# google-deepmind/open_spiel

Hardware: NVIDIA H100
Metric: connect_four ApplyAction env steps/sec (batched) (higher is better)
Workload: dtype u64

## Files before the change

### open_spiel_b200/csrc/api.cu

```cuda
#include <ctype.h>
#include <math.h>
#include <sched.h>
#include <stdlib.h>
#include <stdio.h>
#include <string.h>

#include <memory>
#include <mutex>
#include <string>
#include <vector>

#include "batch_kernels.cuh"
#include "errors.h"

namespace b2s {

long long g_launches = 0;
static thread_local std::string g_err;

int fail(const std::string& m) { g_err = m; return 1; }
int cuda_fail(cudaError_t e, const char* what) {
  g_err = std::string(what) + ": " + cudaGetErrorString(e);
  return 2;
}
#define CU(x) do { cudaError_t _e = (x); if (_e != cudaSuccess) return cuda_fail(_e, #x); } while (0)

constexpr int kMaxDevices = 64;
struct HostPipe {
  std::mutex mu;
  cudaStream_t hs = nullptr, hs2 = nullptr;
  cudaEvent_t ev[8] = {};
};
// ... 134 lines not shown
  if (count == 0) return fail("bind: no CPUs listed in " + path);
  if (sched_setaffinity(0, sizeof set, &set) != 0) return fail("bind: sched_setaffinity failed");
  if (n_cpus) *n_cpus = count;
  return 0;
}

int b2s_device_count(void) {
  int n = 0;
  if (cudaGetDeviceCount(&n) != cudaSuccess) { cudaGetLastError(); return 0; }
  return n;
}

int b2s_batch_create(int game_id, const b2s_params* params, int64_t capacity, int device, void** out_batch) {
  if (!out_batch) return fail("null out_batch");
  *out_batch = nullptr;
  if (capacity <= 0) return fail("capacity must be positive");
  if (b2s_device_count() <= 0) return fail("no CUDA device: the b2s device path has no CPU fallback");
  GameOps* ops = make_ops(game_id, params);
  if (!ops) return fail("unsupported game id");
  b2s_params p;
  if (params) p = *params; else b2s_params_default(&p);
  Batch* B = new Batch;
  B->ops = ops;
  memset(&B->info, 0, sizeof B->info);
  const char* e = ops->configure(p, B->info);
  if (e) { delete B; return fail(e); }
  B->cap = capacity;
  B->device = device;
  cudaError_t ce = cudaSetDevice(device);
  if (ce != cudaSuccess) { delete B; return cuda_fail(ce, "cudaSetDevice"); }
  ops->device_init();
  ce = cudaGetLastError();
  if (ce != cudaSuccess) { delete B; return cuda_fail(ce, "per-game device tables"); }
  size_t bytes = ops->chunk_bytes() * (size_t)ops->chunks() * (size_t)capacity;
  ce = cudaMalloc(&B->planes, bytes);
  if (ce != cudaSuccess) { delete B; return cuda_fail(ce, "cudaMalloc(state planes)"); }
  if (B->info.history_bytes > 0) {
    ce = cudaMalloc((void**)&B->hist, (size_t)B->info.history_bytes * (size_t)capacity);
    if (ce != cudaSuccess) { delete B; return cuda_fail(ce, "cudaMalloc(history)"); }
  }
  ce = cudaMalloc((void**)&B->err, sizeof(ErrBuf));
  if (ce != cudaSuccess) { delete B; return cuda_fail(ce, "cudaMalloc(err)"); }
  ops->reset(B->ctx(), capacity, 0);
  ce = cudaDeviceSynchronize();
  if (ce != cudaSuccess) { delete B; return cuda_fail(ce, "initial reset"); }
  *out_batch = B;
  return 0;
}

void b2s_batch_destroy(void* batch) {
  if (!batch) return;
  Batch* B = (Batch*)batch;
  cudaSetDevice(B->device);
  delete B;
}

int b2s_batch_info(void* batch, b2s_game_info* out) {
  if (!batch || !out) return fail("null argument");
  *out = ((Batch*)batch)->info;
  return 0;
}
int64_t b2s_batch_capacity(void* batch) { return batch ? ((Batch*)batch)->cap : 0; }

int b2s_reset(void* batch, int64_t n, void* stream) {
  if (int r = check(batch, n)) return r;
  Batch* B = (Batch*)batch;
  B->ops->reset(B->ctx(), n, (cudaStream_t)stream);
// ... 36 lines not shown
  Batch* B = (Batch*)batch;
  if (!obs_d) return fail("null obs");
  if ((uintptr_t)obs_d & 3u) return fail("observation: output pointer must be 4-byte aligned");
  if (player >= B->info.num_players) return fail("player out of range");
  const char* e = B->ops->obs(B->ctx(), player, 0, 0, obs_d, n, (cudaStream_t)stream);
  if (e) return fail(e);
  return post();
}

int b2s_information_state(void* batch, int player, float* out_d, int64_t n, void* stream) {
  if (int r = check(batch, n)) return r;
  Batch* B = (Batch*)batch;
  if (!out_d) return fail("null out");
  if ((uintptr_t)out_d & 3u) return fail("information_state: output pointer must be 4-byte aligned");
  if (player >= B->info.num_players) return fail("player out of range");
  const char* e = B->ops->obs(B->ctx(), player, 1, 0, out_d, n, (cudaStream_t)stream);
  if (e) return fail(e);
  return post();
}

int b2s_step_fused(void* batch, const int32_t* actions_d, uint32_t* mask_d, uint8_t* term_d, float* rets_d, int64_t n, void* stream) {
  if (int r = check(batch, n)) return r;
  if (!actions_d) return fail("null actions");
  Batch* B = (Batch*)batch;
  B->ops->step_fused(B->ctx(), actions_d, mask_d, term_d, rets_d, n, (cudaStream_t)stream);
  return post();
}

constexpr size_t kHostGraphsPerBatch = 4;

static int enqueue_host_step(Batch* B, HostPipe& pipe, const void* actions_h, int action_bytes, uint32_t* mask_h, uint8_t* term_or_status_h,
                             float* rets_h, int64_t n, int compact, int n_chunks, bool join) {
  cudaStream_t st = pipe.hs, st2 = pipe.hs2;
  const size_t W = (size_t)B->info.mask_words, P = (size_t)B->info.num_players, cb = B->ops->chunk_bytes();
  const size_t ab = (size_t)action_bytes;
  const int64_t chunk = n_chunks > 1 ? ((n + n_chunks - 1) / n_chunks + 1023) / 1024 * 1024 : n;
  int c = 0, rc = 0;
  cudaError_t e = cudaSuccess;
  for (int64_t lo = 0; lo < n && !rc; lo += chunk, ++c) {
    const int64_t len = n - lo < chunk ? n - lo : chunk;
    Ctx v = B->ctx();
    v.planes = (char*)v.planes + (size_t)lo * cb;
    if (v.hist) v.hist += lo;
    v.lane0 = lo;
    char* act_d = (char*)B->act_d + (size_t)lo * ab;
    e = cudaMemcpyAsync(act_d, (const char*)actions_h + (size_t)lo * ab, ab * len, cudaMemcpyHostToDevice, st);
    if (e != cudaSuccess) { rc = cuda_fail(e, "step_host: upload"); break; }
    if (compact)
      B->ops->step_compact(v, act_d, action_bytes, B->term_d + lo, mask_h ? B->mask_d + lo * W : nullptr, len, st);
    else
      B->ops->step_fused(v, (const int*)act_d, mask_h ? B->mask_d + lo * W : nullptr, term_or_status_h ? B->term_d + lo : nullptr,
                         rets_h ? B->rets_d + lo * P : nullptr, len, st);
    if ((rc = post())) break;
    cudaEvent_t ev = pipe.ev[c % kHostChunks];
    if ((e = cudaEventRecord(ev, st)) != cudaSuccess || (e = cudaStreamWaitEvent(st2, ev, 0)) != cudaSuccess) { rc = cuda_fail(e, "step_host: event"); break; }
    if (mask_h && (e = cudaMemcpyAsync(mask_h + lo * W, B->mask_d + lo * W, sizeof(u32) * W * len, cudaMemcpyDeviceToHost, st2)) != cudaSuccess) { rc = cuda_fail(e, "step_host: download"); break; }
    if (term_or_status_h && (e = cudaMemcpyAsync(term_or_status_h + lo, B->term_d + lo, len, cudaMemcpyDeviceToHost, st2)) != cudaSuccess) { rc = cuda_fail(e, "step_host: download"); break; }
    if (rets_h && (e = cudaMemcpyAsync(rets_h + lo * P, B->rets_d + lo * P, sizeof(float) * P * len, cudaMemcpyDeviceToHost, st2)) != cudaSuccess) { rc = cuda_fail(e, "step_host: download"); break; }
  }
  if (join && c > 0) {
    cudaEvent_t ev = pipe.ev[c % kHostChunks];
    if ((e = cudaEventRecord(ev, st2)) != cudaSuccess || (e = cudaStreamWaitEvent(st, ev, 0)) != cudaSuccess) { if (!rc) rc = cuda_fail(e, "step_host: join"); }
  }
  return rc;
}

static int step_host_impl(Batch* B, const void* actions_h, int action_bytes, uint32_t* mask_h, uint8_t* term_or_status_h,
                          float* rets_h, int64_t n, int compact) {
  if (B->device < 0 || B->device >= kMaxDevices) return fail("device index out of range");
  HostPipe& pipe = g_host_pipe[B->device];
  std::lock_guard<std::mutex> lock(pipe.mu);
  if (!pipe.hs) {
    CU(cudaStreamCreateWithFlags(&pipe.hs, cudaStreamDefault));
    CU(cudaStreamCreateWithFlags(&pipe.hs2, cudaStreamDefault));
    for (int i = 0; i < kHostChunks; ++i) CU(cudaEventCreateWithFlags(&pipe.ev[i], cudaEventDisableTiming));
// ... 105 lines not shown
}

int b2s_step_fused_host_compact(void* batch, const void* actions_h, int action_bytes, uint8_t* status_h, uint32_t* mask_h, int64_t n) {
  if (int r = check(batch, n)) return r;
  if (!actions_h || !status_h) return fail("null actions / status");
  Batch* B = (Batch*)batch;
  if (action_bytes != 1 && action_bytes != 4) return fail("step_compact: action_bytes must be 1 (uint8, 0xFF = skip) or 4 (int32, -1 = skip)");
  if (action_bytes == 1 && B->info.num_distinct_actions > 255) return fail("step_compact: uint8 actions need num_distinct_actions <= 255");
  if (B->info.min_utility != -1.0 || B->info.max_utility != 1.0 || B->info.max_chance_outcomes > 0)
    return fail("step_compact: the 2-bit outcome code needs a win / loss / draw game (use b2s_step_fused_host)");
  return step_host_impl(B, actions_h, action_bytes, mask_h, status_h, nullptr, n, 1);
}

int b2s_error_count(void* batch, int64_t* count, int64_t* first_bad_lane, void* stream) {
  if (int r = check(batch, 0)) return r;
  Batch* B = (Batch*)batch;
  ErrBuf e;
  CU(cudaMemcpyAsync(&e, B->err, sizeof e, cudaMemcpyDeviceToHost, (cudaStream_t)stream));
  CU(cudaStreamSynchronize((cudaStream_t)stream));
  if (count) *count = (int64_t)e.count;
  if (first_bad_lane) *first_bad_lane = e.count ? e.first : -1;
  return 0;
}

int b2s_state_get(void* batch, int64_t idx, void* host_blob, size_t cap) {
  if (int r = check(batch, 0)) return r;
  Batch* B = (Batch*)batch;
  if (idx < 0 || idx >= B->cap) return fail("lane out of range");
  size_t cb = B->ops->chunk_bytes(), sb = (size_t)B->info.state_bytes;
  size_t need = sb + B->info.history_bytes;
  if (cap < need) return fail("blob too small");
  CU(cudaDeviceSynchronize());
  std::vector<uint4> stored((cb * B->ops->chunks() + 15) / 16), blob((sb + 15) / 16);
  for (int k = 0; k < B->ops->chunks(); ++k)
    CU(cudaMemcpy((char*)stored.data() + k * cb, (char*)B->planes + ((size_t)k * B->cap + idx) * cb, cb, cudaMemcpyDeviceToHost));
  B->ops->stored_to_blob(stored.data(), blob.data());
  char* out = (char*)host_blob;
  memcpy(out, blob.data(), sb);
  if (B->info.history_bytes)
    CU(cudaMemcpy2D(out + sb, sizeof(u64), B->hist + idx, sizeof(u64) * B->cap, sizeof(u64),
                    B->info.history_bytes / sizeof(u64), cudaMemcpyDeviceToHost));
  return 0;
}
int b2s_state_set(void* batch, int64_t idx, const void* host_blob, size_t len) {
  if (int r = check(batch, 0)) return r;
  Batch* B = (Batch*)batch;
  if (idx < 0 || idx >= B->cap) return fail("lane out of range");
  size_t cb = B->ops->chunk_bytes(), sb = (size_t)B->info.state_bytes;
  size_t need = sb + B->info.history_bytes;
  if (len != need) return fail("blob size mismatch");
  CU(cudaDeviceSynchronize());
  const char* in = (const char*)host_blob;
  std::vector<uint4> stored((cb * B->ops->chunks() + 15) / 16), blob((sb + 15) / 16);
  memcpy(blob.data(), in, sb);
  B->ops->blob_to_stored(blob.data(), stored.data());
  for (int k = 0; k < B->ops->chunks(); ++k)
    CU(cudaMemcpy((char*)B->planes + ((size_t)k * B->cap + idx) * cb, (const char*)stored.data() + k * cb, cb, cudaMemcpyHostToDevice));
  if (B->info.history_bytes)
    CU(cudaMemcpy2D(B->hist + idx, sizeof(u64) * B->cap, in + sb, sizeof(u64), sizeof(u64),
                    B->info.history_bytes / sizeof(u64), cudaMemcpyHostToDevice));
  return 0;
}

int b2s_broadcast_state(void* dst_batch, int64_t dst_begin, int64_t count, void* src_batch, int64_t src, void* stream) {
  if (int r = check(dst_batch, 0)) return r;
  if (!src_batch) return fail("null src batch");
  Batch* D = (Batch*)dst_batch;
  Batch* S = (Batch*)src_batch;
  if (D->info.game_id != S->info.game_id || D->device != S->device ||
      memcmp(&D->info, &S->info, sizeof(b2s_game_info)) != 0)
    return fail("broadcast: batches differ in game/params/device");
  if (dst_begin < 0 || count < 0 || dst_begin + count > D->cap || src < 0 || src >= S->cap) return fail("broadcast: range");
  D->ops->broadcast(D->ctx(), dst_begin, count, S->ctx(), src, (cudaStream_t)stream);
  return post();
}

int b2s_copy_states(void* dst_batch, int64_t dst_begin, void* src_batch, int64_t src_begin, int64_t count, void* stream) {
  if (int r = check(dst_batch, 0)) return r;
  if (!src_batch) return fail("null src batch");
  Batch* D = (Batch*)dst_batch;
  Batch* S = (Batch*)src_batch;
  if (D->device != S->device || memcmp(&D->info, &S->info, sizeof(b2s_game_info)) != 0)
    return fail("copy: batches differ in game/params/device");
  if (dst_begin < 0 || src_begin < 0 || count < 0 || dst_begin + count > D->cap || src_begin + count > S->cap)
    return fail("copy: range");
  D->ops->copy(D->ctx(), dst_begin, S->ctx(), src_begin, count, (cudaStream_t)stream);
  return post();
}

int b2s_rollout(void* batch, uint64_t seed, int64_t lane_offset, int64_t n, float* rets_d, int32_t* plies_d, void* stream) {
// ... 315 lines not shown
```

### open_spiel_b200/csrc/batch_kernels.cuh

```cuda
#pragma once
#include <new>
#include <string.h>

#include "common.cuh"

namespace b2s {

constexpr int kBlock = 256;

extern long long g_launches;

__device__ __forceinline__ void pdl_wait() { asm volatile("griddepcontrol.wait;" ::: "memory"); }
__device__ __forceinline__ void pdl_launch_dependents() { asm volatile("griddepcontrol.launch_dependents;" ::: "memory"); }

template <typename... KArgs, typename... Args>
inline void launch_pdl(void (*kernel)(KArgs...), unsigned grid, cudaStream_t st, Args... args) {
  cudaLaunchConfig_t cfg = {};
  cfg.gridDim = dim3(grid);
  cfg.blockDim = dim3(kBlock);
  cfg.stream = st;
  cudaLaunchAttribute at[1];
  at[0].id = cudaLaunchAttributeProgrammaticStreamSerialization;
  at[0].val.programmaticStreamSerializationAllowed = 1;
  cfg.attrs = at;
  cfg.numAttrs = 1;
  cudaLaunchKernelEx(&cfg, kernel, static_cast<KArgs>(args)...);
}


template <class R>
__global__ void __launch_bounds__(kBlock) k_reset(Ctx ctx, typename R::Cfg cfg, long long n) {
  long long i = (long long)blockIdx.x * kBlock + threadIdx.x;
  if (i == 0) { ctx.err->count = 0; ctx.err->first = 0x7fffffffffffffffLL; }
  if (i >= n) return;
  typename R::S s;
  R::init(s, cfg, ctx, i);
  store_state<R>(s, cfg, ctx, i);
}

template <class R, int ILP>
__global__ void __launch_bounds__(kBlock, R::kMinBlocks) k_apply(Ctx ctx, typename R::Cfg cfg, const int* __restrict__ actions, long long n) {
  pdl_wait();
  long long base = (long long)blockIdx.x * (kBlock * ILP) + threadIdx.x;
  int a[ILP];
  Fetched<R> pk[ILP];
#pragma unroll
  for (int j = 0; j < ILP; ++j) {
    long long i = base + (long long)j * kBlock;
    a[j] = -1;
    if (i < n) { a[j] = __ldg(actions + i); fetch_state<R>(pk[j], ctx, i); }
  }
  pdl_launch_dependents();
#pragma unroll
  for (int j = 0; j < ILP; ++j) {
    long long i = base + (long long)j * kBlock;
    if (a[j] == -1) continue;
    typename R::S s;
    unpack_state<R>(s, pk[j], cfg);
    if (R::terminal(s, cfg) || !R::apply(s, a[j], cfg, ctx, i)) { flag_error(ctx.err, ctx.lane0 + i); continue; }
    store_state<R>(s, cfg, ctx, i);
  }
}

template <int MAXW>
struct MaskStage {
  static constexpr int kRow = MAXW | 1;
  u32 w[kBlock / 32][32 * kRow];
};
template <int MAXW>
__device__ __forceinline__ void store_masks_coalesced(u32* __restrict__ mask, long long first, long long n, bool active, int W,
                                                      const u32* m, MaskStage<MAXW>& stage) {
  const int lane = threadIdx.x & 31;
  u32* st = stage.w[threadIdx.x >> 5];
  if (active) {
#pragma unroll
    for (int k = 0; k < MAXW; ++k) if (k < W) st[lane * MaskStage<MAXW>::kRow + k] = m[k];
  }
  __syncwarp();
  const long long left = n - first;
  const int total = (int)(left < 32 ? left : 32) * W;
  int q = lane / W, r = lane - q * W;
  const int dq = 32 / W, dr = 32 - dq * W;
  u32* out = mask + first * W;
  for (int f = lane; f < total; f += 32) {
    out[f] = st[q * MaskStage<MAXW>::kRow + r];
    q += dq; r += dr;
    if (r >= W) { r -= W; ++q; }
  }
  __syncwarp();
}

template <class R, int ILP>
__global__ void __launch_bounds__(kBlock) k_legal_mask(Ctx ctx, typename R::Cfg cfg, u32* __restrict__ mask, int mask_words, long long n) {
  long long base = (long long)blockIdx.x * (kBlock * ILP) + threadIdx.x;
  Fetched<R> pk[ILP];
#pragma unroll
  for (int j = 0; j < ILP; ++j) {
    long long i = base + (long long)j * kBlock;
    if (i < n) fetch_state<R>(pk[j], ctx, i);
  }
  __shared__ MaskStage<R::kMaskWords == 1 ? 0 : R::kMaskWords> stage;
#pragma unroll
  for (int j = 0; j < ILP; ++j) {
    long long i = base + (long long)j * kBlock;
    u32 m[R::kMaskWords];
    if (i < n) {
      typename R::S s;
      unpack_state<R>(s, pk[j], cfg);
      R::legal(s, cfg, m);
    }
    if (R::kMaskWords == 1) {
      if (i < n) mask[i] = m[0];
    } else {
      store_masks_coalesced(mask, i - (threadIdx.x & 31), n, i < n, mask_words, m, stage);
    }
  }
}

template <class R>
__global__ void __launch_bounds__(kBlock) k_legal_list(Ctx ctx, typename R::Cfg cfg, short* __restrict__ out, int* __restrict__ counts, int stride, int mask_words, long long n) {
  long long i = (long long)blockIdx.x * kBlock + threadIdx.x;
  if (i >= n) return;
  typename R::S s;
  load_state<R>(s, cfg, ctx, i);
  u32 m[R::kMaskWords];
  R::legal(s, cfg, m);
  int k = 0;
  for (int w = 0; w < mask_words; ++w) {
    u32 bits = m[w];
    while (bits) {
      int b = __ffs(bits) - 1;
      bits &= bits - 1;
      if (k < stride) out[i * stride + k] = (short)(w * 32 + b);
      ++k;
    }
  }
  counts[i] = k;
}

template <class R, int ILP>
__global__ void __launch_bounds__(kBlock) k_status(Ctx ctx, typename R::Cfg cfg, signed char* __restrict__ cur, unsigned char* __restrict__ term, float* __restrict__ rets, long long n) {
  long long base = (long long)blockIdx.x * (kBlock * ILP) + threadIdx.x;
  Fetched<R> pk[ILP];
#pragma unroll
  for (int j = 0; j < ILP; ++j) {
    long long i = base + (long long)j * kBlock;
    if (i < n) fetch_state<R>(pk[j], ctx, i);
  }
#pragma unroll
  for (int j = 0; j < ILP; ++j) {
    long long i = base + (long long)j * kBlock;
    if (i >= n) continue;
    typename R::S s;
    unpack_state<R>(s, pk[j], cfg);
    int cp = R::cur_player(s, cfg);
    if (cur) cur[i] = (signed char)cp;
    if (term) term[i] = cp == kTerminalPlayerId ? 1 : 0;
    if (rets) {
      float r[R::kPlayers];
      R::returns(s, cfg, r);
      if (R::kPlayers == 2) reinterpret_cast<float2*>(rets)[i] = make_float2(r[0], r[1]);
      else { const int np = rule_num_players<R>(cfg); for (int p = 0; p < np; ++p) rets[i * np + p] = r[p]; }
    }
  }
}

template <class R, int ILP>
__global__ void __launch_bounds__(kBlock) k_step_fused(Ctx ctx, typename R::Cfg cfg, const int* __restrict__ actions, u32* __restrict__ mask, int mask_words, unsigned char* __restrict__ term, float* __restrict__ rets, long long n) {
  pdl_wait();
  long long base = (long long)blockIdx.x * (kBlock * ILP) + threadIdx.x;
  int a[ILP];
  Fetched<R> pk[ILP];
#pragma unroll
  for (int j = 0; j < ILP; ++j) {
    long long i = base + (long long)j * kBlock;
    a[j] = -1;
    if (i < n) { a[j] = __ldg(actions + i); fetch_state<R>(pk[j], ctx, i); }
  }
  pdl_launch_dependents();
  __shared__ MaskStage<R::kMaskWords == 1 ? 0 : R::kMaskWords> stage;
#pragma unroll
  for (int j = 0; j < ILP; ++j) {
    long long i = base + (long long)j * kBlock;
    const bool live = i < n;
    u32 m[R::kMaskWords];
    if (live) {
      typename R::S s;
      unpack_state<R>(s, pk[j], cfg);
      if (a[j] != -1) {
        if (R::terminal(s, cfg) || !R::apply(s, a[j], cfg, ctx, i)) flag_error(ctx.err, ctx.lane0 + i);
        else store_state<R>(s, cfg, ctx, i);
      }
      bool t = R::terminal(s, cfg);
      if (term) term[i] = t ? 1 : 0;
      if (rets) {
        float r[R::kPlayers];
        R::returns(s, cfg, r);
        if (R::kPlayers == 2) reinterpret_cast<float2*>(rets)[i] = make_float2(r[0], r[1]);
        else { const int np = rule_num_players<R>(cfg); for (int p = 0; p < np; ++p) rets[i * np + p] = r[p]; }
      }
      if (mask) {
        if (t) { for (int w = 0; w < R::kMaskWords; ++w) m[w] = 0; }
        else R::legal_nonterminal(s, cfg, m);
      }
    }
    if (mask) {
      if (R::kMaskWords == 1) { if (live) mask[i] = m[0]; }
      else store_masks_coalesced(mask, i - (threadIdx.x & 31), n, live, mask_words, m, stage);
    }
  }
}

template <class R, int ILP, class AT>
__global__ void __launch_bounds__(kBlock) k_step_compact(Ctx ctx, typename R::Cfg cfg, const AT* __restrict__ actions, unsigned char* __restrict__ status,
                                                         u32* __restrict__ mask, int mask_words, int small_mask, long long n) {
  pdl_wait();
  long long base = (long long)blockIdx.x * (kBlock * ILP) + threadIdx.x;
  int a[ILP];
  Fetched<R> pk[ILP];
#pragma unroll
  for (int j = 0; j < ILP; ++j) {
    long long i = base + (long long)j * kBlock;
    a[j] = -1;
    if (i < n) {
      AT raw = __ldg(actions + i);
      a[j] = (sizeof(AT) == 1 && (unsigned char)raw == 0xFFu) ? -1 : (int)raw;
      fetch_state<R>(pk[j], ctx, i);
    }
  }
  pdl_launch_dependents();
  __shared__ MaskStage<R::kMaskWords == 1 ? 0 : R::kMaskWords> stage;
#pragma unroll
  for (int j = 0; j < ILP; ++j) {
    long long i = base + (long long)j * kBlock;
    const bool live = i < n;
    u32 m[R::kMaskWords];
    if (live) {
      typename R::S s;
      unpack_state<R>(s, pk[j], cfg);
      if (a[j] != -1) {
        if (R::terminal(s, cfg) || !R::apply(s, a[j], cfg, ctx, i)) flag_error(ctx.err, ctx.lane0 + i);
        else store_state<R>(s, cfg, ctx, i);
// ... 269 lines not shown
__global__ void __launch_bounds__(kBlock) k_copy_to_blob(Ctx dst, Ctx srcctx, long long count, typename R::Cfg cfg) {
  long long i = (long long)blockIdx.x * kBlock + threadIdx.x;
  if (i >= count) return;
  typename R::S s;
  load_state<R>(s, cfg, srcctx, i);
  R::store(s, dst, i);
  R::copy_history(dst, i, srcctx, i, s, cfg);
}

template <class R>
__global__ void __launch_bounds__(kBlock) k_gather(Ctx dst, Ctx srcctx, const long long* __restrict__ src_lanes, long long count, typename R::Cfg cfg) {
  long long i = (long long)blockIdx.x * kBlock + threadIdx.x;
  if (i >= count) return;
  long long sl = src_lanes[i];
  if (sl < 0 || sl >= srcctx.cap) { flag_error(dst.err, i); return; }
  typename R::S s;
  load_state<R>(s, cfg, srcctx, sl);
  store_state<R>(s, cfg, dst, i);
  R::copy_history(dst, i, srcctx, sl, s, cfg);
}


struct Batch;

template <class R> auto call_device_init(int) -> decltype(R::device_init(), void()) { R::device_init(); }
template <class R> void call_device_init(long) {}

struct GameOps {
  virtual ~GameOps() {}
  virtual void device_init() = 0;
  virtual const char* configure(const b2s_params& p, b2s_game_info& gi) = 0;
  virtual size_t chunk_bytes() const = 0;
  virtual int chunks() const = 0;
  virtual void stored_to_blob(const void* stored, void* blob) const = 0;
  virtual void blob_to_stored(const void* blob, void* stored) const = 0;
  virtual void reset(const Ctx&, long long n, cudaStream_t) = 0;
  virtual void apply(const Ctx&, const int* a, long long n, cudaStream_t) = 0;
  virtual void legal_mask(const Ctx&, u32* m, long long n, cudaStream_t) = 0;
  virtual void legal_list(const Ctx&, short* out, int* counts, int stride, long long n, cudaStream_t) = 0;
  virtual void status(const Ctx&, signed char* cur, unsigned char* term, float* rets, long long n, cudaStream_t) = 0;
  virtual const char* obs(const Ctx&, int player, int which, int zero_terminal, float* out, long long n, cudaStream_t) = 0;
  virtual void step_fused(const Ctx&, const int* a, u32* m, unsigned char* term, float* rets, long long n, cudaStream_t) = 0;
  virtual void step_compact(const Ctx&, const void* a, int action_bytes, unsigned char* status, u32* m, long long n, cudaStream_t) = 0;
  virtual void step_compact_zero_copy(const Ctx&, const unsigned char* a_host, unsigned char* status_host, long long n, cudaStream_t) = 0;
  virtual void rollout(const Ctx&, u64 seed, long long lane_offset, float* rets, int* plies, long long n, cudaStream_t) = 0;
  virtual void broadcast(const Ctx& dst, long long dst0, long long count, const Ctx& src, long long srclane, cudaStream_t) = 0;
  virtual void copy(const Ctx& dst, long long dst0, const Ctx& src, long long src0, long long count, cudaStream_t) = 0;
  virtual void copy_to_blob(const Ctx& dst, const Ctx& src, long long count, cudaStream_t) = 0;
  virtual void gather(const Ctx& dst, const Ctx& src, const long long* src_lanes, long long count, cudaStream_t) = 0;
  virtual void traj_begin(const Ctx&, u64 seed, long long lane_offset, int* lengths, long long n, cudaStream_t) = 0;
  virtual void traj_step(const Ctx&, u64 seed, long long lane_offset, int t, const TrajStepOut& o, long long n, cudaStream_t) = 0;
  virtual void traj_finish(const Ctx&, float* rewards, long long n, cudaStream_t) = 0;
  virtual const char* mcts(const Ctx& roots, const Ctx& work, long long n, const struct MctsArgs& args, cudaStream_t) = 0;
  virtual const char* mcts_eval_limits(int* max_legal, int* max_path) const = 0;
  virtual void mcts_eval_step(const Ctx& roots, const Ctx& leaves, long long n, const struct MctsEvalArgs& args, cudaStream_t) = 0;
  virtual void mcts_eval_report(long long n, const struct MctsEvalArgs& args, cudaStream_t) = 0;
  b2s_game_info info;
};

template <class R, class Q = typename R::Packed>
void stored_to_blob_impl(const typename R::Cfg& c, const void* stored, void* blob, int) {
  typename R::S s;
  R::unpack(s, *static_cast<const Q*>(stored), c);
  Ctx b = {};
  b.planes = blob; b.cap = 1;
  R::store(s, b, 0);
// ... 11 lines not shown
template <class R>
void blob_to_stored_impl(const typename R::Cfg&, const void* blob, void* stored, long) { memcpy(stored, blob, sizeof(typename R::Chunk) * R::kChunks); }

inline unsigned grid_for(long long n, int ilp = 1) { return (unsigned)((n + (long long)kBlock * ilp - 1) / ((long long)kBlock * ilp)); }

inline bool make_magic(int d, int limit, u32* out) {
  u64 M = ((1ull << 32) + d - 1) / d;
  if (M >> 32) { if (d == 1) { *out = 0; return false; } }
  for (int e = 0; e < limit; ++e)
    if ((int)(((u64)e * M) >> 32) != e / d) return false;
  *out = (u32)M;
  return true;
}

template <class R>
struct GameOpsT : GameOps {
  typename R::Cfg cfg;
  const char* configure(const b2s_params& p, b2s_game_info& gi) override {
    const char* e = R::make_cfg(p, cfg, gi);
    if (e) return e;
    int width = gi.num_distinct_actions > gi.max_chance_outcomes ? gi.num_distinct_actions : gi.max_chance_outcomes;
    gi.mask_words = (width + 31) / 32;
    if (gi.mask_words > R::kMaskWords) return "action space too large for the device path";
    gi.state_bytes = (int)(sizeof(typename R::Chunk) * R::kChunks);
    gi.game_id = R::kGameId;
    info = gi;
    return nullptr;
  }
  void device_init() override { call_device_init<R>(0); }
  size_t chunk_bytes() const override { return sizeof(StoredChunk<R>); }
  void stored_to_blob(const void* stored, void* blob) const override { stored_to_blob_impl<R>(cfg, stored, blob, 0); }
  void blob_to_stored(const void* blob, void* stored) const override { blob_to_stored_impl<R>(cfg, blob, stored, 0); }
  int chunks() const override { return R::kChunks; }
  void reset(const Ctx& c, long long n, cudaStream_t st) override {
    long long m = n > 0 ? n : 1;
    k_reset<R><<<grid_for(m), kBlock, 0, st>>>(c, cfg, n); ++g_launches;
  }
  void apply(const Ctx& c, const int* a, long long n, cudaStream_t st) override {
    if (n <= 0) return;
    launch_pdl(k_apply<R, R::kIlp>, grid_for(n, R::kIlp), st, c, cfg, a, n); ++g_launches;
  }
  void legal_mask(const Ctx& c, u32* m, long long n, cudaStream_t st) override {
    if (n <= 0) return;
    k_legal_mask<R, R::kIlp><<<grid_for(n, R::kIlp), kBlock, 0, st>>>(c, cfg, m, info.mask_words, n); ++g_launches;
  }
  void legal_list(const Ctx& c, short* out, int* counts, int stride, long long n, cudaStream_t st) override {
    if (n <= 0) return;
    k_legal_list<R><<<grid_for(n), kBlock, 0, st>>>(c, cfg, out, counts, stride, info.mask_words, n); ++g_launches;
  }
  void status(const Ctx& c, signed char* cur, unsigned char* term, float* rets, long long n, cudaStream_t st) override {
    if (n <= 0) return;
    k_status<R, R::kIlp><<<grid_for(n, R::kIlp), kBlock, 0, st>>>(c, cfg, cur, term, rets, n); ++g_launches;
  }
  const char* obs(const Ctx& c, int player, int which, int zero_terminal, float* out, long long n, cudaStream_t st) override {
    int size = which == 0 ? info.observation_tensor_size : info.information_state_tensor_size;
    if (size <= 0) return "game provides no such tensor";
    if (which == 1 && !R::kHasInfoState) return "game provides no information state tensor";
    if (n <= 0) return nullptr;
    u32 magic;
    if (!make_magic(size, 32 * size, &magic)) return "internal: no division magic";
    k_obs<R><<<grid_for(n), kBlock, 0, st>>>(c, cfg, player, which, zero_terminal, out, size, magic, n); ++g_launches;
    return nullptr;
  }
  void step_fused(const Ctx& c, const int* a, u32* m, unsigned char* term, float* rets, long long n, cudaStream_t st) override {
    if (n <= 0) return;
    launch_pdl(k_step_fused<R, R::kIlp>, grid_for(n, R::kIlp), st, c, cfg, a, m, info.mask_words, term, rets, n); ++g_launches;
// ... 126 lines not shown
```

### open_spiel_b200/csrc/common.cuh

```cuda
#pragma once
#include <cuda_runtime.h>
#include <stdint.h>

#include "../../include/b2s.h"

namespace b2s {

typedef unsigned long long u64;
typedef unsigned int u32;

constexpr int kChancePlayerId = -1;
constexpr int kTerminalPlayerId = -4;

struct ErrBuf {
  u64 count;
  long long first;
};

__device__ __forceinline__ void flag_error(ErrBuf* e, long long lane) {
  atomicAdd(&e->count, 1ull);
  atomicMin(&e->first, lane);
}

struct Ctx {
// ... 36 lines not shown
      if ((u32)m >= n || (u32)m >= (u32)(0u - n) % n) return (u32)(m >> 32);
    }
  }
}

__device__ __forceinline__ int nth_set_bit(const u32* words, int nwords, int k) {
  for (int w = 0; w < nwords; ++w) {
    int c = __popc(words[w]);
    if (k < c) return w * 32 + (int)__fns(words[w], 0, k + 1);
    k -= c;
  }
  return -1;
}

template <class R, class S, class Cfg>
__device__ __forceinline__ auto apply_known_legal_impl(S& s, int a, const Cfg& c, const Ctx& ctx, long long lane, int)
    -> decltype(R::apply_legal(s, a, c, ctx, lane)) { return R::apply_legal(s, a, c, ctx, lane); }
template <class R, class S, class Cfg>
__device__ __forceinline__ bool apply_known_legal_impl(S& s, int a, const Cfg& c, const Ctx& ctx, long long lane, long) {
  return R::apply(s, a, c, ctx, lane);
}
template <class R, class S, class Cfg>
__device__ __forceinline__ bool apply_known_legal(S& s, int a, const Cfg& c, const Ctx& ctx, long long lane) {
  return apply_known_legal_impl<R>(s, a, c, ctx, lane, 0);
}

template <class R, class Cfg>
__device__ __forceinline__ auto rule_num_players_impl(const Cfg& c, int) -> decltype(R::num_players(c)) { return R::num_players(c); }
template <class R, class Cfg>
__device__ __forceinline__ int rule_num_players_impl(const Cfg&, long) { return R::kPlayers; }
template <class R, class Cfg>
__device__ __forceinline__ int rule_num_players(const Cfg& c) { return rule_num_players_impl<R>(c, 0); }

template <class R> auto fetched_of(int) -> typename R::Packed;
template <class R> auto fetched_of(long) -> typename R::S;
template <class R> using Fetched = decltype(fetched_of<R>(0));
template <class R> auto stored_of(int) -> typename R::Packed;
template <class R> auto stored_of(long) -> typename R::Chunk;
template <class R> using StoredChunk = decltype(stored_of<R>(0));
template <class R, class P, class Q = typename R::Packed>
__device__ __forceinline__ void fetch_state_impl(P& p, const Ctx& ctx, long long i, int) { p = reinterpret_cast<const Q*>(ctx.planes)[i]; }
template <class R, class P>
__device__ __forceinline__ void fetch_state_impl(P& p, const Ctx& ctx, long long i, long) { R::load(p, ctx, i); }
template <class R, class P>
__device__ __forceinline__ void fetch_state(P& p, const Ctx& ctx, long long i) { fetch_state_impl<R>(p, ctx, i, 0); }
template <class R, class S, class P, class Cfg, class Q = typename R::Packed>
__device__ __forceinline__ void unpack_state_impl(S& s, const P& p, const Cfg& c, int) { R::unpack(s, p, c); }
template <class R, class S, class P, class Cfg>
__device__ __forceinline__ void unpack_state_impl(S& s, const P& p, const Cfg&, long) { s = p; }
template <class R, class S, class P, class Cfg>
__device__ __forceinline__ void unpack_state(S& s, const P& p, const Cfg& c) { unpack_state_impl<R>(s, p, c, 0); }
template <class R, class S, class Cfg, class Q = typename R::Packed>
__device__ __forceinline__ void load_state_impl(S& s, const Cfg& c, const Ctx& ctx, long long i, int) {
  R::unpack(s, reinterpret_cast<const Q*>(ctx.planes)[i], c);
}
template <class R, class S, class Cfg>
__device__ __forceinline__ void load_state_impl(S& s, const Cfg&, const Ctx& ctx, long long i, long) { R::load(s, ctx, i); }
template <class R, class S, class Cfg>
__device__ __forceinline__ void load_state(S& s, const Cfg& c, const Ctx& ctx, long long i) { load_state_impl<R>(s, c, ctx, i, 0); }
template <class R, class S, class Cfg, class Q = typename R::Packed>
__device__ __forceinline__ void store_state_impl(const S& s, const Cfg& c, const Ctx& ctx, long long i, int) {
  reinterpret_cast<Q*>(ctx.planes)[i] = R::pack(s, c);
}
template <class R, class S, class Cfg>
__device__ __forceinline__ void store_state_impl(const S& s, const Cfg&, const Ctx& ctx, long long i, long) { R::store(s, ctx, i); }
template <class R, class S, class Cfg>
__device__ __forceinline__ void store_state(const S& s, const Cfg& c, const Ctx& ctx, long long i) { store_state_impl<R>(s, c, ctx, i, 0); }

template <class R, class S, class Cfg, class Draw>
__device__ __forceinline__ auto playout_step_impl(S& s, const Cfg& c, const Ctx& ctx, long long lane, int ,
                                                  Draw& draw, u32 ply, int) -> decltype(R::num_candidates(s, c)) {
  int n = R::num_candidates(s, c);
  for (u32 retry = 0;; ++retry) {
    int a = R::candidate(s, c, (int)draw(ply + 4096u * retry, (u32)n));
    if (R::play_candidate(s, a, c, ctx, lane)) return a;
  }
}
template <class R, class S, class Cfg, class Draw>
__device__ __forceinline__ int playout_step_impl(S& s, const Cfg& c, const Ctx& ctx, long long lane, int mask_words,
                                                 Draw& draw, u32 ply, long) {
  u32 m[R::kMaskWords];
  R::legal_nonterminal(s, c, m);
  int cnt = 0;
  for (int w = 0; w < mask_words; ++w) cnt += __popc(m[w]);
  int a = nth_set_bit(m, mask_words, (int)draw(ply, (u32)cnt));
  apply_known_legal<R>(s, a, c, ctx, lane);
  return a;
}
template <class R, class S, class Cfg, class Draw>
__device__ __forceinline__ int playout_step(S& s, const Cfg& c, const Ctx& ctx, long long lane, int mask_words, Draw& draw, u32 ply) {
  return playout_step_impl<R>(s, c, ctx, lane, mask_words, draw, ply, 0);
}

struct B128 {
  u64 lo, hi;
// ... 134 lines not shown
```

### open_spiel_b200/csrc/rules_connect_four.cuh

```cuda
#pragma once
#include "common.cuh"

namespace b2s {

template <bool kStd>
struct ConnectFourCore {
  static constexpr int kGameId = B2S_CONNECT_FOUR;
  typedef uint4 Chunk;
  typedef u64 Packed;
  static constexpr int kChunks = 1;
  static constexpr int kMaskWords = 1;
  static constexpr int kObsWords = 3;
  static constexpr int kPlayers = 2;
  static constexpr int kMaxPath = 72;
  static constexpr int kMaxLegal = 32;
  static constexpr int kFilterWords = 0;
  static constexpr int kIlp = 4;
  static constexpr int kMinBlocks = 6;
  static constexpr bool kHasInfoState = false;
  static constexpr int kStdRows = 6, kStdCols = 7, kStdK = 4;

  struct Cfg {
    int rows, cols, k, ego;
    int h1;
    int meta;
    int gather;
    u32 gmul_lo, gmul_hi;
    int gsh_lo, gsh_hi, cols_lo;
    int rgather;
    u32 rmul_lo, rmul_hi;
    int rsh_lo, rsh_hi, rcols_lo, rfirst_hi;
    u64 top;
    u64 board;
    u64 bottom;
    u64 fill[6];
  };
  struct S { u64 x, o; };
  __host__ __device__ static __forceinline__ int ROWS(const Cfg& c) { return kStd ? kStdRows : c.rows; }
  __host__ __device__ static __forceinline__ int COLS(const Cfg& c) { return kStd ? kStdCols : c.cols; }
  __host__ __device__ static __forceinline__ int H1(const Cfg& c) { return kStd ? kStdRows + 1 : c.h1; }
  __host__ __device__ static __forceinline__ int K(const Cfg& c) { return kStd ? kStdK : c.k; }
  __host__ __device__ static __forceinline__ bool META(const Cfg& c) { return kStd ? true : c.meta != 0; }

  static __host__ const char* make_cfg(const b2s_params& p, Cfg& c, b2s_game_info& gi) {
    c.rows = p.rows >= 0 ? p.rows : 6;
    c.cols = p.columns >= 0 ? p.columns : 7;
    c.k = p.x_in_row >= 0 ? p.x_in_row : 4;
    c.ego = p.egocentric_obs_tensor > 0 ? 1 : 0;
    if (c.rows < 1 || c.cols < 1 || c.k < 1) return "connect_four: rows, columns, x_in_row must be positive";
    if ((c.rows + 1) * c.cols > 64 || c.cols > 32)
      return "connect_four: (rows+1)*columns must fit 64 bits for the device path";
    if (kStd && (c.rows != kStdRows || c.cols != kStdCols || c.k != kStdK)) return "connect_four: not the default board";
// ... 234 lines not shown
```

Before: 139.4 billion.

## Store standard connect-four state in 7-byte lane tiles with quad-lane vector access

Standard connect-four states are stored in a tiled layout of 128 lanes per 896 bytes (4-byte low word, 2-byte and 1-byte high planes) instead of 8 bytes per lane. Each thread now owns four consecutive lanes and reads or writes them with vectorized loads and stores for actions, state, masks, terminal flags and returns. The aim is to cut memory traffic in this bandwidth-bound step kernel. In exchange it adds byte-permute pack and unpack work, special handling at the batch tail, and tiled host-side lane read/write paths.

```diff
diff --git a/open_spiel_b200/csrc/api.cu b/open_spiel_b200/csrc/api.cu
--- a/open_spiel_b200/csrc/api.cu
+++ b/open_spiel_b200/csrc/api.cu
@@ -1,3 +1,4 @@
+#include <cassert>
 #include <ctype.h>
 #include <math.h>
 #include <sched.h>
@@ -198,7 +199,7 @@
   ops->device_init();
   ce = cudaGetLastError();
   if (ce != cudaSuccess) { delete B; return cuda_fail(ce, "per-game device tables"); }
-  size_t bytes = ops->chunk_bytes() * (size_t)ops->chunks() * (size_t)capacity;
+  size_t bytes = ops->planes_bytes(capacity);
   ce = cudaMalloc(&B->planes, bytes);
   if (ce != cudaSuccess) { delete B; return cuda_fail(ce, "cudaMalloc(state planes)"); }
   if (B->info.history_bytes > 0) {
@@ -301,7 +302,7 @@
 static int enqueue_host_step(Batch* B, HostPipe& pipe, const void* actions_h, int action_bytes, uint32_t* mask_h, uint8_t* term_or_status_h,
                              float* rets_h, int64_t n, int compact, int n_chunks, bool join) {
   cudaStream_t st = pipe.hs, st2 = pipe.hs2;
-  const size_t W = (size_t)B->info.mask_words, P = (size_t)B->info.num_players, cb = B->ops->chunk_bytes();
+  const size_t W = (size_t)B->info.mask_words, P = (size_t)B->info.num_players;
   const size_t ab = (size_t)action_bytes;
   const int64_t chunk = n_chunks > 1 ? ((n + n_chunks - 1) / n_chunks + 1023) / 1024 * 1024 : n;
   int c = 0, rc = 0;
@@ -309,7 +310,8 @@
   for (int64_t lo = 0; lo < n && !rc; lo += chunk, ++c) {
     const int64_t len = n - lo < chunk ? n - lo : chunk;
     Ctx v = B->ctx();
-    v.planes = (char*)v.planes + (size_t)lo * cb;
+    assert(lo % 1024 == 0);
+    v.planes = (char*)v.planes + B->ops->lane_offset(lo);
     if (v.hist) v.hist += lo;
     v.lane0 = lo;
     char* act_d = (char*)B->act_d + (size_t)lo * ab;
@@ -481,8 +483,7 @@
   if (cap < need) return fail("blob too small");
   CU(cudaDeviceSynchronize());
   std::vector<uint4> stored((cb * B->ops->chunks() + 15) / 16), blob((sb + 15) / 16);
-  for (int k = 0; k < B->ops->chunks(); ++k)
-    CU(cudaMemcpy((char*)stored.data() + k * cb, (char*)B->planes + ((size_t)k * B->cap + idx) * cb, cb, cudaMemcpyDeviceToHost));
+  CU(B->ops->read_lane(B->planes, B->cap, idx, stored.data()));
   B->ops->stored_to_blob(stored.data(), blob.data());
   char* out = (char*)host_blob;
   memcpy(out, blob.data(), sb);
@@ -503,8 +504,7 @@
   std::vector<uint4> stored((cb * B->ops->chunks() + 15) / 16), blob((sb + 15) / 16);
   memcpy(blob.data(), in, sb);
   B->ops->blob_to_stored(blob.data(), stored.data());
-  for (int k = 0; k < B->ops->chunks(); ++k)
-    CU(cudaMemcpy((char*)B->planes + ((size_t)k * B->cap + idx) * cb, (const char*)stored.data() + k * cb, cb, cudaMemcpyHostToDevice));
+  CU(B->ops->write_lane(B->planes, B->cap, idx, stored.data()));
   if (B->info.history_bytes)
     CU(cudaMemcpy2D(B->hist + idx, sizeof(u64) * B->cap, in + sb, sizeof(u64), sizeof(u64),
                     B->info.history_bytes / sizeof(u64), cudaMemcpyHostToDevice));
diff --git a/open_spiel_b200/csrc/batch_kernels.cuh b/open_spiel_b200/csrc/batch_kernels.cuh
--- a/open_spiel_b200/csrc/batch_kernels.cuh
+++ b/open_spiel_b200/csrc/batch_kernels.cuh
@@ -28,6 +28,44 @@
 }
 
 
+template <class AT>
+__device__ __forceinline__ int action_of(AT raw) { return (sizeof(AT) == 1 && (unsigned char)raw == 0xFFu) ? -1 : (int)raw; }
+template <class AT>
+__device__ __forceinline__ void actions4(int a[4], const AT* __restrict__ act, long long i0, long long n) {
+  if (i0 + 4 <= n && ((unsigned long long)(act + i0) & (4 * sizeof(AT) - 1)) == 0) {
+    if constexpr (sizeof(AT) == 4) {
+      const int4 v = __ldg(reinterpret_cast<const int4*>(act + i0));
+      a[0] = v.x; a[1] = v.y; a[2] = v.z; a[3] = v.w;
+    } else {
+      const uchar4 v = __ldg(reinterpret_cast<const uchar4*>(act + i0));
+      a[0] = action_of(v.x); a[1] = action_of(v.y); a[2] = action_of(v.z); a[3] = action_of(v.w);
+    }
+  } else {
+#pragma unroll
+    for (int j = 0; j < 4; ++j) a[j] = i0 + j < n ? action_of(__ldg(act + i0 + j)) : -1;
+  }
+}
+__device__ __forceinline__ void out4(u32* __restrict__ p, long long i0, long long n, const u32 v[4]) {
+  if (i0 + 4 <= n && ((unsigned long long)(p + i0) & 15) == 0) *reinterpret_cast<uint4*>(p + i0) = make_uint4(v[0], v[1], v[2], v[3]);
+  else for (int j = 0; j < 4; ++j) if (i0 + j < n) p[i0 + j] = v[j];
+}
+__device__ __forceinline__ void out4(unsigned char* __restrict__ p, long long i0, long long n, const u32 v[4]) {
+  if (i0 + 4 <= n && ((unsigned long long)(p + i0) & 3) == 0) *reinterpret_cast<u32*>(p + i0) = v[0] | v[1] << 8 | v[2] << 16 | v[3] << 24;
+  else for (int j = 0; j < 4; ++j) if (i0 + j < n) p[i0 + j] = (unsigned char)v[j];
+}
+__device__ __forceinline__ void out4(float2* __restrict__ p, long long i0, long long n, const float2 v[4]) {
+  if (i0 + 4 <= n && ((unsigned long long)(p + i0) & 15) == 0) {
+    reinterpret_cast<float4*>(p + i0)[0] = make_float4(v[0].x, v[0].y, v[1].x, v[1].y);
+    reinterpret_cast<float4*>(p + i0)[1] = make_float4(v[2].x, v[2].y, v[3].x, v[3].y);
+  } else for (int j = 0; j < 4; ++j) if (i0 + j < n) p[i0 + j] = v[j];
+}
+template <class R, int ILP>
+__device__ __forceinline__ long long stream_base() {
+  if constexpr (lane_tiled<R>()) return 4 * ((long long)blockIdx.x * kBlock + threadIdx.x);
+  else return (long long)blockIdx.x * (kBlock * ILP) + threadIdx.x;
+}
+template <class R> constexpr long long stream_stride() { return lane_tiled<R>() ? 1 : kBlock; }
+
 template <class R>
 __global__ void __launch_bounds__(kBlock) k_reset(Ctx ctx, typename R::Cfg cfg, long long n) {
   long long i = (long long)blockIdx.x * kBlock + threadIdx.x;
@@ -40,26 +78,37 @@
 
 template <class R, int ILP>
 __global__ void __launch_bounds__(kBlock, R::kMinBlocks) k_apply(Ctx ctx, typename R::Cfg cfg, const int* __restrict__ actions, long long n) {
+  constexpr bool Q = lane_tiled<R>();
+  static_assert(!Q || ILP == 4, "a thread owns one quad of tiled lanes");
   pdl_wait();
-  long long base = (long long)blockIdx.x * (kBlock * ILP) + threadIdx.x;
+  const long long base = stream_base<R, ILP>();
+  constexpr long long kStride = stream_stride<R>();
   int a[ILP];
   Fetched<R> pk[ILP];
+  if constexpr (Q) {
+    actions4(a, actions, base, n);
+    lanes4_fetch(pk, ctx, base, n);
+  } else {
+#pragma unroll
+    for (int j = 0; j < ILP; ++j) {
+      long long i = base + (long long)j * kStride;
+      a[j] = -1;
+      if (i < n) { a[j] = __ldg(actions + i); fetch_state<R>(pk[j], ctx, i); }
+    }
+  }
+  pdl_launch_dependents();
+  unsigned moved = 0;
 #pragma unroll
   for (int j = 0; j < ILP; ++j) {
-    long long i = base + (long long)j * kBlock;
-    a[j] = -1;
-    if (i < n) { a[j] = __ldg(actions + i); fetch_state<R>(pk[j], ctx, i); }
-  }
-  pdl_launch_dependents();
-#pragma unroll
-  for (int j = 0; j < ILP; ++j) {
-    long long i = base + (long long)j * kBlock;
+    long long i = base + (long long)j * kStride;
     if (a[j] == -1) continue;
     typename R::S s;
     unpack_state<R>(s, pk[j], cfg);
     if (R::terminal(s, cfg) || !R::apply(s, a[j], cfg, ctx, i)) { flag_error(ctx.err, ctx.lane0 + i); continue; }
-    store_state<R>(s, cfg, ctx, i);
-  }
+    if constexpr (Q) { pk[j] = R::pack(s, cfg); moved |= 1u << j; }
+    else store_state<R>(s, cfg, ctx, i);
+  }
+  if constexpr (Q) lanes4_store(pk, moved, ctx, base, n);
 }
 
 template <int MAXW>
@@ -92,29 +141,38 @@
 
 template <class R, int ILP>
 __global__ void __launch_bounds__(kBlock) k_legal_mask(Ctx ctx, typename R::Cfg cfg, u32* __restrict__ mask, int mask_words, long long n) {
-  long long base = (long long)blockIdx.x * (kBlock * ILP) + threadIdx.x;
+  constexpr bool Q = lane_tiled<R>();
+  static_assert(!Q || (ILP == 4 && R::kMaskWords == 1), "a thread owns one quad of tiled lanes");
+  const long long base = stream_base<R, ILP>();
+  constexpr long long kStride = stream_stride<R>();
   Fetched<R> pk[ILP];
+  if constexpr (Q) lanes4_fetch(pk, ctx, base, n);
+  else {
+#pragma unroll
+    for (int j = 0; j < ILP; ++j) {
+      long long i = base + (long long)j * kStride;
+      if (i < n) fetch_state<R>(pk[j], ctx, i);
+    }
+  }
+  __shared__ MaskStage<R::kMaskWords == 1 ? 0 : R::kMaskWords> stage;
+  u32 m4[4];
 #pragma unroll
   for (int j = 0; j < ILP; ++j) {
-    long long i = base + (long long)j * kBlock;
-    if (i < n) fetch_state<R>(pk[j], ctx, i);
-  }
-  __shared__ MaskStage<R::kMaskWords == 1 ? 0 : R::kMaskWords> stage;
-#pragma unroll
-  for (int j = 0; j < ILP; ++j) {
-    long long i = base + (long long)j * kBlock;
+    long long i = base + (long long)j * kStride;
     u32 m[R::kMaskWords];
     if (i < n) {
       typename R::S s;
       unpack_state<R>(s, pk[j], cfg);
       R::legal(s, cfg, m);
     }
-    if (R::kMaskWords == 1) {
+    if constexpr (Q) m4[j] = m[0];
+    else if (R::kMaskWords == 1) {
       if (i < n) mask[i] = m[0];
     } else {
       store_masks_coalesced(mask, i - (threadIdx.x & 31), n, i < n, mask_words, m, stage);
     }
   }
+  if constexpr (Q) out4(mask, base, n, m4);
 }
 
 template <class R>
@@ -140,20 +198,34 @@
 
 template <class R, int ILP>
 __global__ void __launch_bounds__(kBlock) k_status(Ctx ctx, typename R::Cfg cfg, signed char* __restrict__ cur, unsigned char* __restrict__ term, float* __restrict__ rets, long long n) {
-  long long base = (long long)blockIdx.x * (kBlock * ILP) + threadIdx.x;
+  constexpr bool Q = lane_tiled<R>();
+  static_assert(!Q || (ILP == 4 && R::kPlayers == 2), "a thread owns one quad of tiled lanes");
+  const long long base = stream_base<R, ILP>();
+  constexpr long long kStride = stream_stride<R>();
   Fetched<R> pk[ILP];
+  if constexpr (Q) lanes4_fetch(pk, ctx, base, n);
+  else {
+#pragma unroll
+    for (int j = 0; j < ILP; ++j) {
+      long long i = base + (long long)j * kStride;
+      if (i < n) fetch_state<R>(pk[j], ctx, i);
+    }
+  }
+  u32 cp4[4] = {0, 0, 0, 0}, t4[4] = {0, 0, 0, 0};
+  float2 r4[4] = {};
 #pragma unroll
   for (int j = 0; j < ILP; ++j) {
-    long long i = base + (long long)j * kBlock;
-    if (i < n) fetch_state<R>(pk[j], ctx, i);
-  }
-#pragma unroll
-  for (int j = 0; j < ILP; ++j) {
-    long long i = base + (long long)j * kBlock;
+    long long i = base + (long long)j * kStride;
     if (i >= n) continue;
     typename R::S s;
     unpack_state<R>(s, pk[j], cfg);
     int cp = R::cur_player(s, cfg);
+    if constexpr (Q) {
+      cp4[j] = (unsigned char)(signed char)cp; t4[j] = cp == kTerminalPlayerId ? 1 : 0;
+      float r[R::kPlayers];
+      if (rets) { R::returns(s, cfg, r); r4[j] = make_float2(r[0], r[1]); }
+      continue;
+    }
     if (cur) cur[i] = (signed char)cp;
     if (term) term[i] = cp == kTerminalPlayerId ? 1 : 0;
     if (rets) {
@@ -163,25 +235,41 @@
       else { const int np = rule_num_players<R>(cfg); for (int p = 0; p < np; ++p) rets[i * np + p] = r[p]; }
     }
   }
+  if constexpr (Q) {
+    if (cur) out4(reinterpret_cast<unsigned char*>(cur), base, n, cp4);
+    if (term) out4(term, base, n, t4);
+    if (rets) out4(reinterpret_cast<float2*>(rets), base, n, r4);
+  }
 }
 
 template <class R, int ILP>
 __global__ void __launch_bounds__(kBlock) k_step_fused(Ctx ctx, typename R::Cfg cfg, const int* __restrict__ actions, u32* __restrict__ mask, int mask_words, unsigned char* __restrict__ term, float* __restrict__ rets, long long n) {
+  constexpr bool Q = lane_tiled<R>();
+  static_assert(!Q || (ILP == 4 && R::kMaskWords == 1 && R::kPlayers == 2), "a thread owns one quad of tiled lanes");
   pdl_wait();
-  long long base = (long long)blockIdx.x * (kBlock * ILP) + threadIdx.x;
+  const long long base = stream_base<R, ILP>();
+  constexpr long long kStride = stream_stride<R>();
   int a[ILP];
   Fetched<R> pk[ILP];
-#pragma unroll
-  for (int j = 0; j < ILP; ++j) {
-    long long i = base + (long long)j * kBlock;
-    a[j] = -1;
-    if (i < n) { a[j] = __ldg(actions + i); fetch_state<R>(pk[j], ctx, i); }
+  if constexpr (Q) {
+    actions4(a, actions, base, n);
+    lanes4_fetch(pk, ctx, base, n);
+  } else {
+#pragma unroll
+    for (int j = 0; j < ILP; ++j) {
+      long long i = base + (long long)j * kStride;
+      a[j] = -1;
+      if (i < n) { a[j] = __ldg(actions + i); fetch_state<R>(pk[j], ctx, i); }
+    }
   }
   pdl_launch_dependents();
   __shared__ MaskStage<R::kMaskWords == 1 ? 0 : R::kMaskWords> stage;
+  unsigned moved = 0, tb = 0;
+  u32 m4[4] = {0, 0, 0, 0};
+  float2 r4[4] = {};
 #pragma unroll
   for (int j = 0; j < ILP; ++j) {
-    long long i = base + (long long)j * kBlock;
+    long long i = base + (long long)j * kStride;
     const bool live = i < n;
     u32 m[R::kMaskWords];
     if (live) {
@@ -189,9 +277,16 @@
       unpack_state<R>(s, pk[j], cfg);
       if (a[j] != -1) {
         if (R::terminal(s, cfg) || !R::apply(s, a[j], cfg, ctx, i)) flag_error(ctx.err, ctx.lane0 + i);
+        else if constexpr (Q) { pk[j] = R::pack(s, cfg); moved |= 1u << j; }
         else store_state<R>(s, cfg, ctx, i);
       }
       bool t = R::terminal(s, cfg);
+      if constexpr (Q) {
+        tb |= (t ? 1u : 0u) << (8 * j);
+        if (rets) { float r[R::kPlayers]; R::returns(s, cfg, r); r4[j] = make_float2(r[0], r[1]); }
+        if (mask) { if (t) m4[j] = 0; else { R::legal_nonterminal(s, cfg, m); m4[j] = m[0]; } }
+        continue;
+      }
       if (term) term[i] = t ? 1 : 0;
       if (rets) {
         float r[R::kPlayers];
@@ -204,10 +299,19 @@
         else R::legal_nonterminal(s, cfg, m);
       }
     }
-    if (mask) {
-      if (R::kMaskWords == 1) { if (live) mask[i] = m[0]; }
-      else store_masks_coalesced(mask, i - (threadIdx.x & 31), n, live, mask_words, m, stage);
-    }
+    if constexpr (!Q) {
+      if (mask) {
+        if (R::kMaskWords == 1) { if (live) mask[i] = m[0]; }
+        else store_masks_coalesced(mask, i - (threadIdx.x & 31), n, live, mask_words, m, stage);
+      }
+    }
+  }
+  if constexpr (Q) {
+    lanes4_store(pk, moved, ctx, base, n);
+    const u32 t4[4] = {tb & 0xFFu, (tb >> 8) & 0xFFu, (tb >> 16) & 0xFFu, tb >> 24};
+    if (term) out4(term, base, n, t4);
+    if (rets) out4(reinterpret_cast<float2*>(rets), base, n, r4);
+    if (mask) out4(mask, base, n, m4);
   }
 }
 
@@ -543,6 +647,10 @@
   virtual const char* configure(const b2s_params& p, b2s_game_info& gi) = 0;
   virtual size_t chunk_bytes() const = 0;
   virtual int chunks() const = 0;
+  virtual size_t planes_bytes(long long lanes) const = 0;
+  virtual size_t lane_offset(long long lo) const = 0;
+  virtual cudaError_t read_lane(const void* planes, long long cap, long long idx, void* stored) const = 0;
+  virtual cudaError_t write_lane(void* planes, long long cap, long long idx, const void* stored) const = 0;
   virtual void stored_to_blob(const void* stored, void* blob) const = 0;
   virtual void blob_to_stored(const void* blob, void* stored) const = 0;
   virtual void reset(const Ctx&, long long n, cudaStream_t) = 0;
@@ -620,6 +728,54 @@
   void stored_to_blob(const void* stored, void* blob) const override { stored_to_blob_impl<R>(cfg, stored, blob, 0); }
   void blob_to_stored(const void* blob, void* stored) const override { blob_to_stored_impl<R>(cfg, blob, stored, 0); }
   int chunks() const override { return R::kChunks; }
+  size_t planes_bytes(long long lanes) const override {
+    if constexpr (lane_tiled<R>()) return tile7_bytes(lanes);
+    else return sizeof(StoredChunk<R>) * (size_t)R::kChunks * (size_t)lanes;
+  }
+  size_t lane_offset(long long lo) const override {
+    if constexpr (lane_tiled<R>()) return tile7_bytes(lo);
+    else return sizeof(StoredChunk<R>) * (size_t)lo;
+  }
+  cudaError_t read_lane(const void* planes, long long cap, long long idx, void* stored) const override {
+    if constexpr (lane_tiled<R>()) {
+      const char* t = (const char*)planes + (idx >> 7) * 896;
+      const int sl = (int)(idx & 127);
+      u32 lo = 0; unsigned short b45 = 0; unsigned char b6 = 0;
+      cudaError_t e = cudaMemcpy(&lo, t + 4 * sl, 4, cudaMemcpyDeviceToHost);
+      if (e == cudaSuccess) e = cudaMemcpy(&b45, t + 512 + 2 * sl, 2, cudaMemcpyDeviceToHost);
+      if (e == cudaSuccess) e = cudaMemcpy(&b6, t + 768 + sl, 1, cudaMemcpyDeviceToHost);
+      *static_cast<u64*>(stored) = (u64)lo | (u64)tile7_hi(b45, b6) << 32;
+      return e;
+    } else {
+      const size_t cb = sizeof(StoredChunk<R>);
+      for (int k = 0; k < R::kChunks; ++k) {
+        cudaError_t e = cudaMemcpy((char*)stored + k * cb, (const char*)planes + ((size_t)k * cap + idx) * cb, cb, cudaMemcpyDeviceToHost);
+        if (e != cudaSuccess) return e;
+      }
+      return cudaSuccess;
+    }
+  }
+  cudaError_t write_lane(void* planes, long long cap, long long idx, const void* stored) const override {
+    if constexpr (lane_tiled<R>()) {
+      char* t = (char*)planes + (idx >> 7) * 896;
+      const int sl = (int)(idx & 127);
+      const u64 key = *static_cast<const u64*>(stored);
+      const u32 lo = (u32)key, hi = (u32)(key >> 32);
+      const unsigned short b45 = (unsigned short)hi;
+      const unsigned char b6 = (unsigned char)tile7_b6(hi);
+      cudaError_t e = cudaMemcpy(t + 4 * sl, &lo, 4, cudaMemcpyHostToDevice);
+      if (e == cudaSuccess) e = cudaMemcpy(t + 512 + 2 * sl, &b45, 2, cudaMemcpyHostToDevice);
+      if (e == cudaSuccess) e = cudaMemcpy(t + 768 + sl, &b6, 1, cudaMemcpyHostToDevice);
+      return e;
+    } else {
+      const size_t cb = sizeof(StoredChunk<R>);
+      for (int k = 0; k < R::kChunks; ++k) {
+        cudaError_t e = cudaMemcpy((char*)planes + ((size_t)k * cap + idx) * cb, (const char*)stored + k * cb, cb, cudaMemcpyHostToDevice);
+        if (e != cudaSuccess) return e;
+      }
+      return cudaSuccess;
+    }
+  }
   void reset(const Ctx& c, long long n, cudaStream_t st) override {
     long long m = n > 0 ? n : 1;
     k_reset<R><<<grid_for(m), kBlock, 0, st>>>(c, cfg, n); ++g_launches;
diff --git a/open_spiel_b200/csrc/common.cuh b/open_spiel_b200/csrc/common.cuh
--- a/open_spiel_b200/csrc/common.cuh
+++ b/open_spiel_b200/csrc/common.cuh
@@ -92,6 +92,57 @@
 template <class R, class Cfg>
 __device__ __forceinline__ int rule_num_players(const Cfg& c) { return rule_num_players_impl<R>(c, 0); }
 
+template <class R> constexpr auto tiled_of(int) -> decltype(R::kTiled7) { return R::kTiled7; }
+template <class R> constexpr bool tiled_of(long) { return false; }
+template <class R> constexpr bool lane_tiled() { return tiled_of<R>(0); }
+__host__ __device__ __forceinline__ size_t tile7_bytes(long long lanes) { return (size_t)((lanes + 127) >> 7) * 896; }
+__host__ __device__ __forceinline__ u32 tile7_hi(u32 b45, u32 b6) { return (b45 | b6 << 16 | b6 << 24) & 0xC001FFFFu; }
+__host__ __device__ __forceinline__ u32 tile7_b6(u32 hi) { return ((hi >> 16) | (hi >> 24)) & 0xFFu; }
+__host__ __device__ __forceinline__ u64 tile7_get(const void* planes, long long i) {
+  const unsigned char* t = static_cast<const unsigned char*>(planes) + (i >> 7) * 896;
+  const int s = (int)(i & 127);
+  return (u64)reinterpret_cast<const u32*>(t)[s] | (u64)tile7_hi(reinterpret_cast<const unsigned short*>(t + 512)[s], t[768 + s]) << 32;
+}
+__host__ __device__ __forceinline__ void tile7_set(void* planes, long long i, u64 key) {
+  unsigned char* t = static_cast<unsigned char*>(planes) + (i >> 7) * 896;
+  const int s = (int)(i & 127);
+  const u32 hi = (u32)(key >> 32);
+  reinterpret_cast<u32*>(t)[s] = (u32)key;
+  reinterpret_cast<unsigned short*>(t + 512)[s] = (unsigned short)hi;
+  t[768 + s] = (unsigned char)tile7_b6(hi);
+}
+__device__ __forceinline__ void lanes4_fetch(u64 k[4], const Ctx& ctx, long long i0, long long n) {
+  if (i0 + 4 <= n) {
+    const unsigned char* t = static_cast<const unsigned char*>(ctx.planes) + (i0 >> 7) * 896;
+    const int w = (int)((i0 & 127) >> 2);
+    const uint4 a = reinterpret_cast<const uint4*>(t)[w];
+    const uint2 b = reinterpret_cast<const uint2*>(t + 512)[w];
+    const u32 c = reinterpret_cast<const u32*>(t + 768)[w];
+    k[0] = (u64)a.x | (u64)(__byte_perm(b.x, c, 0x4410) & 0xC001FFFFu) << 32;
+    k[1] = (u64)a.y | (u64)(__byte_perm(b.x, c, 0x5532) & 0xC001FFFFu) << 32;
+    k[2] = (u64)a.z | (u64)(__byte_perm(b.y, c, 0x6610) & 0xC001FFFFu) << 32;
+    k[3] = (u64)a.w | (u64)(__byte_perm(b.y, c, 0x7732) & 0xC001FFFFu) << 32;
+  } else {
+#pragma unroll
+    for (int j = 0; j < 4; ++j) if (i0 + j < n) k[j] = tile7_get(ctx.planes, i0 + j);
+  }
+}
+__device__ __forceinline__ void lanes4_store(const u64 k[4], unsigned moved, const Ctx& ctx, long long i0, long long n) {
+  if (!moved) return;
+  if (i0 + 4 <= n) {
+    unsigned char* t = static_cast<unsigned char*>(ctx.planes) + (i0 >> 7) * 896;
+    const int w = (int)((i0 & 127) >> 2);
+    const u32 h0 = (u32)(k[0] >> 32), h1 = (u32)(k[1] >> 32), h2 = (u32)(k[2] >> 32), h3 = (u32)(k[3] >> 32);
+    const u32 t0 = h0 | h0 >> 8, t1 = h1 | h1 >> 8, t2 = h2 | h2 >> 8, t3 = h3 | h3 >> 8;
+    reinterpret_cast<uint4*>(t)[w] = make_uint4((u32)k[0], (u32)k[1], (u32)k[2], (u32)k[3]);
+    reinterpret_cast<uint2*>(t + 512)[w] = make_uint2(__byte_perm(h0, h1, 0x5410), __byte_perm(h2, h3, 0x5410));
+    reinterpret_cast<u32*>(t + 768)[w] = __byte_perm(__byte_perm(t0, t1, 0x0062), __byte_perm(t2, t3, 0x0062), 0x5410);
+  } else {
+#pragma unroll
+    for (int j = 0; j < 4; ++j) if (((moved >> j) & 1u) && i0 + j < n) tile7_set(ctx.planes, i0 + j, k[j]);
+  }
+}
+
 template <class R> auto fetched_of(int) -> typename R::Packed;
 template <class R> auto fetched_of(long) -> typename R::S;
 template <class R> using Fetched = decltype(fetched_of<R>(0));
@@ -99,7 +150,10 @@
 template <class R> auto stored_of(long) -> typename R::Chunk;
 template <class R> using StoredChunk = decltype(stored_of<R>(0));
 template <class R, class P, class Q = typename R::Packed>
-__device__ __forceinline__ void fetch_state_impl(P& p, const Ctx& ctx, long long i, int) { p = reinterpret_cast<const Q*>(ctx.planes)[i]; }
+__device__ __forceinline__ void fetch_state_impl(P& p, const Ctx& ctx, long long i, int) {
+  if constexpr (lane_tiled<R>()) p = tile7_get(ctx.planes, i);
+  else p = reinterpret_cast<const Q*>(ctx.planes)[i];
+}
 template <class R, class P>
 __device__ __forceinline__ void fetch_state_impl(P& p, const Ctx& ctx, long long i, long) { R::load(p, ctx, i); }
 template <class R, class P>
@@ -112,7 +166,8 @@
 __device__ __forceinline__ void unpack_state(S& s, const P& p, const Cfg& c) { unpack_state_impl<R>(s, p, c, 0); }
 template <class R, class S, class Cfg, class Q = typename R::Packed>
 __device__ __forceinline__ void load_state_impl(S& s, const Cfg& c, const Ctx& ctx, long long i, int) {
-  R::unpack(s, reinterpret_cast<const Q*>(ctx.planes)[i], c);
+  if constexpr (lane_tiled<R>()) R::unpack(s, tile7_get(ctx.planes, i), c);
+  else R::unpack(s, reinterpret_cast<const Q*>(ctx.planes)[i], c);
 }
 template <class R, class S, class Cfg>
 __device__ __forceinline__ void load_state_impl(S& s, const Cfg&, const Ctx& ctx, long long i, long) { R::load(s, ctx, i); }
@@ -120,7 +175,8 @@
 __device__ __forceinline__ void load_state(S& s, const Cfg& c, const Ctx& ctx, long long i) { load_state_impl<R>(s, c, ctx, i, 0); }
 template <class R, class S, class Cfg, class Q = typename R::Packed>
 __device__ __forceinline__ void store_state_impl(const S& s, const Cfg& c, const Ctx& ctx, long long i, int) {
-  reinterpret_cast<Q*>(ctx.planes)[i] = R::pack(s, c);
+  if constexpr (lane_tiled<R>()) tile7_set(ctx.planes, i, R::pack(s, c));
+  else reinterpret_cast<Q*>(ctx.planes)[i] = R::pack(s, c);
 }
 template <class R, class S, class Cfg>
 __device__ __forceinline__ void store_state_impl(const S& s, const Cfg&, const Ctx& ctx, long long i, long) { R::store(s, ctx, i); }
diff --git a/open_spiel_b200/csrc/rules_connect_four.cuh b/open_spiel_b200/csrc/rules_connect_four.cuh
--- a/open_spiel_b200/csrc/rules_connect_four.cuh
+++ b/open_spiel_b200/csrc/rules_connect_four.cuh
@@ -18,6 +18,7 @@
   static constexpr int kIlp = 4;
   static constexpr int kMinBlocks = 6;
   static constexpr bool kHasInfoState = false;
+  static constexpr bool kTiled7 = kStd;
   static constexpr int kStdRows = 6, kStdCols = 7, kStdK = 4;
 
   struct Cfg {
```

After: 143.8 billion (median of 6 runs). +3.1%, better.
